# Aazmp/vp8oclenc

Hardware: AMD Instinct MI355X
Metric: macroblocks/sec inter-frame (ME+DCT+loopfilter), 1080p (higher is better)
Workload: dtype u8/int32

## Files before the change

vp8oclenc_amd/csrc/kernels_s2.hip:

```cpp
#include <stdlib.h>
#include <string.h>

#include "vp8hip_dev.h"
#include "kernels_rc_dev.h"

namespace vp8 {

namespace {

constexpr uint32_t pk8(int a, int b, int c, int d) {
    return (uint32_t)(a & 255) | ((uint32_t)(b & 255) << 8) | ((uint32_t)(c & 255) << 16) | ((uint32_t)(d & 255) << 24);
}
constexpr int TAPS[5][6] = {{3, -16, 77, 77, -16, 3}, {1, -8, 36, 108, -11, 2}, {0, 0, 128, 0, 0, 0}, {2, -11, 108, 36, -8, 1}, {3, -16, 77, 77, -16, 3}};
struct OperandTable { uint32_t w[64][4]; };
constexpr OperandTable make_bh() {
    OperandTable t{};
    for (int l = 0; l < 64; ++l) {
        const int n = l & 31, xi = n >> 3, c = n & 7, xc = xi + (xi >> 1), s = xc >= 2 ? 1 : 0;
        for (int j = 0; j < 16; ++j) {
            const int k = 16 * (l >> 5) + j, tap = k - c - s;
            const int v = k == 31 ? 64 : (tap >= 0 && tap < 6) ? TAPS[xc][tap] : 0;
            t.w[l][j >> 2] |= (uint32_t)(v & 255) << (8 * (j & 3));
        }
    }
    return t;
}
constexpr OperandTable make_av() {
    OperandTable t{};
    for (int l = 0; l < 64; ++l) {
        const int m = l & 31, f = m >> 3, i = m & 7, yc = f + (f >> 1), s = yc >= 2 ? 1 : 0;
        for (int j = 0; j < 16; ++j) {
            const int k = 16 * (l >> 5) + j, tap = k - i - s;
            const int v = k == 31 ? 64 : (tap >= 0 && tap < 6) ? TAPS[yc][tap] : 0;
            t.w[l][j >> 2] |= (uint32_t)(v & 255) << (8 * (j & 3));
        }
    }
    return t;
}
static __device__ __constant__ const OperandTable K_BH = make_bh();
static __device__ __constant__ const OperandTable K_AV = make_av();

constexpr int HT_XC = 36;
constexpr int V_CAND = 4;
constexpr int V_ROW = 26 * V_CAND;
constexpr int V_SLOT = 4 * V_ROW;
constexpr int V_ZERO = 25;
constexpr int PRE_SLOT = 96;
constexpr int WIN_ROW = 8;
__device__ __forceinline__ void lds_fence() { asm volatile("s_waitcnt lgkmcnt(0)" ::: "memory"); }

struct S2Args {
    Plane cur;
    Plane ref[3];
    const int16_t *net_in[3];
    int16_t *net_out[3];
    int32_t *bdiff[3];
    int refmap[3];
    int nrefs;
    int w, h, nblk, bw;
    uint32_t bw_inv;
    unsigned long long *clk;
};

__device__ __forceinline__ uint32_t umin(uint32_t a, uint32_t b) { return a < b ? a : b; }
template <int CTRL, int ROW_MASK = 0xf>
__device__ __forceinline__ uint32_t dpp(uint32_t v) {
    return (uint32_t)__builtin_amdgcn_update_dpp((int)v, (int)v, CTRL, ROW_MASK, 0xf, false);
}
template <int CTRL, int ROW_MASK = 0xf>
__device__ __forceinline__ uint32_t dpp_or_max(uint32_t v) {
    return (uint32_t)__builtin_amdgcn_update_dpp(-1, (int)v, CTRL, ROW_MASK, 0xf, false);
}
__device__ __forceinline__ uint32_t halfwave_min_upper(uint32_t key) {
    key = umin(key, dpp_or_max<0xb1>(key));
    key = umin(key, dpp_or_max<0x4e>(key));
    key = umin(key, dpp_or_max<0x141>(key));
    key = umin(key, dpp_or_max<0x140>(key));
    return umin(key, dpp_or_max<0x142, 0xa>(key));
}

typedef unsigned short us2 __attribute__((ext_vector_type(2)));
__device__ __forceinline__ unsigned short ashr7_pk_i8(int a, int b) { return __builtin_amdgcn_ashr_pk_i8_i32(a, b, 7); }
__device__ __forceinline__ uint32_t pack4(unsigned short lo, unsigned short hi) {
    const us2 v = {lo, hi};
    return __builtin_bit_cast(uint32_t, v);
}
__device__ __forceinline__ uint32_t round_pack4(const v16i &acc, int q) {
    return pack4(ashr7_pk_i8(acc[4 * q], acc[4 * q + 1]), ashr7_pk_i8(acc[4 * q + 2], acc[4 * q + 3]));
}
__device__ __forceinline__ v4i one_at_k31(v4i d, int upper) {
    d.w = (int)(((uint32_t)d.w & (0xffffffffu >> (8 & upper))) | (0x01000000u & (uint32_t)upper));
    return d;
}
__device__ __forceinline__ v16i mfma_round(v4i a, v4i b) {
    const v16i c = {0, 0, 0, 0, 0, 0, 0, 0, 0, 0, 0, 0, 0, 0, 0, 0};
    return __builtin_amdgcn_mfma_i32_32x32x32_i8(a, b, c, 0, 0, 0);
}

template <bool SPREAD, bool ALLREFS>
__device__ __forceinline__ void search2_body(const S2Args &a, int wg_x, int ref_idx, int tn) {
    if (ALLREFS ? a.nrefs == 0 : ref_idx >= a.nrefs) return;
    __shared__ __attribute__((aligned(16))) uint32_t s_HT[8][5 * HT_XC];
    __shared__ __attribute__((aligned(16))) uint32_t s_V[8][V_SLOT];
    uint32_t(*s_win)[V_SLOT] = s_V;
    __shared__ __attribute__((aligned(16))) int s_pre[8][PRE_SLOT];
    int(*s_q3)[5 * HT_XC] = reinterpret_cast<int(*)[5 * HT_XC]>(s_HT);
    const int g = threadIdx.x >> 5, lane = threadIdx.x & 31;
    const int wl = threadIdx.x & 63, kh = wl >> 5, gp = g & ~1;
    const int b = imin(wg_x * 8 + g, a.nblk - 1);
    const bool live = wg_x * 8 + g < a.nblk;
    const int by = a.bw == 1 ? b : (int)__umulhi((uint32_t)b, a.bw_inv), bx = b - by * a.bw;
    const int cx = bx * 8, cy = by * 8;
    {
        const int g_n = tn >> 5, lane_n = tn & 31;
        uint32_t *tmp = reinterpret_cast<uint32_t *>(&s_pre[g_n][80]);
        if (lane_n < 16) {
            const int row = lane_n >> 1, half = lane_n & 1;
            const uint32_t v = *reinterpret_cast<const uint32_t *>(a.cur.p + (ptrdiff_t)(cy + row) * a.cur.stride + cx + 4 * half) ^ 0x80808080u;
            uint8_t *cz = reinterpret_cast<uint8_t *>(tmp) + (row >> 2) * 32 + half * 16 + (row & 3);
#pragma unroll
            for (int j = 0; j < 4; ++j) cz[j * 4] = (uint8_t)(v >> (8 * j));
        }
        lds_fence();
        const int hf = lane_n & 1, t = imin(lane_n >> 1, 5), qb = imin(t, 3);
        const v4i cv = *reinterpret_cast<const v4i *>(tmp + 4 * qb);
        const uint32_t cc[4] = {(uint32_t)cv.x, (uint32_t)cv.y, (uint32_t)cv.z, (uint32_t)cv.w};
        int smcd[4], xy[4];
        weight_pre_half(cc, hf ? K_W_R2 : K_W_R0, hf ? K_W_Y : K_W_X, smcd, xy);
        int *dst = &s_pre[g_n][16 * t + 4 * hf];
        *reinterpret_cast<v4i *>(dst) = v4i{smcd[0], smcd[1], smcd[2], smcd[3]};
        *reinterpret_cast<v4i *>(dst + METRIC_X) = v4i{xy[0], xy[1], xy[2], xy[3]};
    }
    const int k = lane;
    const int dx = k % 5 - 2, dy = k / 5 - 2;
    const uint32_t kcode = k < 25 ? (uint32_t)((iabs(dx) + iabs(dy)) * 32 * 256 + (dy + 2) * 8 + dx + 2) : 40u;
    const v4i wa = metric_a(wl);

    auto one_reference = [&](int ri) {
        int tr = tn;
        if (ALLREFS) asm volatile("" : "+v"(tr));
        const int g_n = tr >> 5, lane_n = tr & 31, wl_n = tr & 63, kh_n = wl_n >> 5, gp_n = g_n & ~1;
        const int r = a.refmap[ri];
        const uint32_t nv = reinterpret_cast<const uint32_t *>(a.net_in[r])[b];
        const int nx = (int16_t)(nv & 0xffffu), ny = (int16_t)(nv >> 16);
        const int v0x = (int16_t)(nx * 4), v0y = (int16_t)(ny * 4);
        const int Lx = iclamp(cx + nx, 3 - EXT, a.w + EXT - 11), Ly = iclamp(cy + ny, 3 - EXT, a.h + EXT - 11);
        const Plane rf = a.ref[r];
        {
            const int row = lane_n >> 1, half = lane_n & 1;
            v4i v;
            __builtin_memcpy(&v, rf.p + (ptrdiff_t)(Ly - 3 + row) * rf.stride + (Lx - 3) + 16 * half, 16);
            *reinterpret_cast<v4i *>(&s_win[g_n][row * WIN_ROW + 4 * half]) = v ^ (int)0x80808080u;
        }
        const uint32_t zv = *reinterpret_cast<const uint32_t *>(rf.p + (ptrdiff_t)(cy + ((lane_n >> 1) & 7)) * rf.stride + cx + 4 * (lane_n & 1)) ^ 0x80808080u;
        lds_fence();

        {
            const int m = wl & 31, m_n = wl_n & 31;
            const v4i aw = *reinterpret_cast<const v4i *>(&s_win[gp_n + (m_n >> 4)][(m_n & 15) * WIN_ROW + 4 * kh_n]);
            const v4i bh = *reinterpret_cast<const v4i *>(K_BH.w[wl_n]);
            const v16i acc = mfma_round(one_at_k31(aw, -kh_n), bh);
            const int xi = m >> 3, c = m & 7, xc = xi + (xi >> 1);
            uint32_t *ht = &s_HT[gp][xc * HT_XC + c * 4 + kh];
#pragma unroll
            for (int q = 0; q < 4; ++q) ht[(q >> 1) * (5 * HT_XC) + 2 * (q & 1)] = round_pack4(acc, q);
        }
        {
            const int c = lane_n & 7, rg = lane_n >> 3;
            const uint8_t *wb = reinterpret_cast<const uint8_t *>(s_win[g_n]) + 3 + c + rg * (16 * WIN_ROW);
            uint32_t v = 0;
#pragma unroll
            for (int rr = 0; rr < 4; ++rr) v |= (uint32_t)wb[rr * (4 * WIN_ROW)] << (8 * rr);
            s_HT[g_n][2 * HT_XC + c * 4 + rg] = v;
        }
        {
            const int row = (lane_n >> 1) & 7, half = lane_n & 1;
            uint8_t *z = reinterpret_cast<uint8_t *>(&s_V[g_n][((row >> 2) * 2 + half) * V_ROW + V_ZERO * V_CAND]) + (row & 3);
#pragma unroll
            for (int j = 0; j < 4; ++j) z[j * 4] = (uint8_t)(zv >> (8 * j));
        }
        lds_fence();

        {
            const v4i av = *reinterpret_cast<const v4i *>(K_AV.w[wl_n]);
#pragma unroll
            for (int t = 0; t < 3; ++t) {
                const int ng = 32 * t + (wl & 31);
                const bool on = t < 2 || (wl & 31) < 16;
                const int blk = ng >= 40 ? 1 : 0, rem = on ? ng - 40 * blk : 0, xc = rem >> 3, c = rem & 7;
                const v4i hv = *reinterpret_cast<const v4i *>(&s_HT[gp + blk][xc * HT_XC + c * 4]);
                const v16i acc = mfma_round(av, one_at_k31(hv, -kh_n));
                if (on) {
                    uint32_t *sv = &s_V[gp + blk][(kh * 2 + (c >> 2)) * V_ROW + xc * V_CAND + (c & 3)];
#pragma unroll
                    for (int f = 0; f < 4; ++f) sv[(f + (f >> 1)) * 5 * V_CAND] = round_pack4(acc, f);
                    sv[2 * 5 * V_CAND] = kh ? __builtin_amdgcn_alignbyte((uint32_t)hv[2], (uint32_t)hv[1], 3)
                                            : __builtin_amdgcn_alignbyte((uint32_t)hv[1], (uint32_t)hv[0], 3);
                }
            }
        }
        lds_fence();

        int qx = (int16_t)(cx * 4 + v0x + dx), qy = (int16_t)(cy * 4 + v0y + dy);
        if (k == 25) { qx = cx * 4; qy = cy * 4; }
        const bool valid = live && k < 26 && qx >= 0 && qx <= a.w * 4 - 32 && qy >= 0 && qy <= a.h * 4 - 32;
        int diff = 0;
        auto metric = [&](const uint32_t *src, const int *pre16) { return weight_mfma(wa, load_pre16(pre16), *reinterpret_cast<const v4i *>(src)); };
        if (SPREAD) {
            int *q3 = &s_q3[g][64];
            const bool helper = lane >= 26;
            const uint32_t *src = helper ? &s_V[g][3 * V_ROW + (lane - 26) * 3 * V_CAND] : &s_V[g][k * V_CAND];
            const int step = helper ? V_CAND : V_ROW;
            const int *pre = &s_pre[g][helper ? 48 : 0];
            int *dst = &q3[helper ? (lane - 26) * 3 : 29];
#pragma unroll
            for (int j = 0; j < 3; ++j) {
                const int c = metric(src + j * step, pre + 16 * j);
                dst[j] = c;
                diff += c;
            }
            __syncthreads();
            if ((int)(threadIdx.x >> 6) == (wg_x & 3)) {
                const int slot = wl >> 3, cand = 18 + (wl & 7);
                s_q3[slot][64 + cand] = metric(&s_V[slot][3 * V_ROW + cand * V_CAND], &s_pre[slot][48]);
            }
            __syncthreads();
            diff += q3[k < 26 ? k : 31];
        } else {
            const uint32_t *src = &s_V[g][imin(k, V_ZERO) * V_CAND];
#pragma unroll
            for (int bb = 0; bb < 4; ++bb) diff += metric(src + bb * V_ROW, &s_pre[g][bb * 16]);
        }
        uint32_t key = ((uint32_t)diff << 8) + kcode;
        key = (valid && key < (0x7fffu << 8)) ? key : 0xffffffffu;
        key = halfwave_min_upper(key);
        if (lane == 16 && live) {
            int vx = (int16_t)((int16_t)(a.w * 4 - 32) - cx * 4), vy = (int16_t)((int16_t)(a.h * 4 - 32) - cy * 4), md = 0x7fff;
            if (key != 0xffffffffu) {
                const int kk = key & 0xff;
                md = (int)(key >> 8);
                vx = kk == 40 ? 0 : (int16_t)(v0x + (kk & 7) - 2);
                vy = kk == 40 ? 0 : (int16_t)(v0y + (kk >> 3) - 2);
            }
            if ((vx != 0) | (vy != 0)) md -= (iabs(vx - v0x) + iabs(vy - v0y)) * 32;
            reinterpret_cast<uint32_t *>(a.net_out[r])[b] = (uint32_t)(uint16_t)vx | ((uint32_t)(uint16_t)vy << 16);
            a.bdiff[r][b] = md;
        }
    };
    if (ALLREFS) {
#pragma unroll 1
        for (int ri = 0; ri < a.nrefs; ++ri) one_reference(ri);
    } else {
        one_reference(ref_idx);
    }
}

template <bool SPREAD, int ITER, bool ALLREFS>
__device__ __forceinline__ void search2_groups(const S2Args &a, int grp, int ref_idx) {
    if (ITER == 1 && !ALLREFS) { search2_body<SPREAD, ALLREFS>(a, grp, ref_idx, (int)threadIdx.x); return; }
#pragma unroll 1
    for (int it = 0; it < ITER; ++it) {
        int tn = (int)threadIdx.x;
        asm volatile("" : "+v"(tn));
        search2_body<SPREAD, ALLREFS>(a, grp * ITER + it, ref_idx, tn);
    }
}
template <bool SPREAD, int ITER>
__global__ __attribute__((amdgpu_waves_per_eu(7, 8))) __launch_bounds__(256) void k_search2(S2Args a) {
    launch_clock_begin(a.clk);
    search2_groups<SPREAD, ITER, false>(a, xcd_band(blockIdx.x, gridDim.x), blockIdx.y);
    launch_clock_end(a.clk);
}
static_assert(sizeof(BatchOf<S2Args>) <= 4096, "a batch's argument blocks travel in the 4 KiB kernel-argument segment");
template <bool SPREAD, int ITER>
__global__ __attribute__((amdgpu_waves_per_eu(7, 8))) __launch_bounds__(256) void k_search2_b(BatchOf<S2Args> b) {
    launch_clock_begin(b.item[0].clk);
    search2_groups<SPREAD, ITER, true>(b.item[blockIdx.z], xcd_band(blockIdx.x, gridDim.x), 0);
    launch_clock_end(b.item[0].clk);
}
struct S2Scans { rc::ScanCore item[MAX_BATCH]; uint32_t mask; int nbx, wgs; };
static_assert(sizeof(BatchOf<S2Args>) + sizeof(S2Scans) <= 4096, "the kernel-argument segment");
template <bool SPREAD, int ITER>
__global__ __attribute__((amdgpu_waves_per_eu(7, 8))) __launch_bounds__(256) void k_search2_bs(BatchOf<S2Args> b, S2Scans sc) {
    if ((int)blockIdx.x >= sc.nbx) {
        const int wg = (int)blockIdx.x - sc.nbx;
        if (((sc.mask >> blockIdx.z) & 1) && wg < sc.wgs) rc::strength_segments_body(b.item[blockIdx.z].cur, sc.item[blockIdx.z], wg, sc.wgs);
        return;
    }
    launch_clock_begin(b.item[0].clk);
    search2_groups<SPREAD, ITER, true>(b.item[blockIdx.z], xcd_band(blockIdx.x, sc.nbx), 0);
    launch_clock_end(b.item[0].clk);
}
__global__ __launch_bounds__(256, 4) void k_search2_p(BatchOf<S2Args> b, int nbx, int maxrefs, int total) {
    for (int w = blockIdx.x; w < total; w += gridDim.x) {
        const int item = w / (nbx * maxrefs), rem = w - item * (nbx * maxrefs);
        const int ref_idx = rem / nbx, wg_x = rem - ref_idx * nbx;
        search2_body<false, false>(b.item[item], wg_x, ref_idx, (int)threadIdx.x);
        lds_fence();
    }
}

}

static S2Args search2_args(const Frame &cur, const RefSet &refs, const NetSet &nets, unsigned long long *clk) {
    S2Args a;
    a.clk = clk;
    a.cur = cur.Y[0];
    int n = 0;
    for (int r = 0; r < 3; ++r) {
        a.ref[r] = refs.ref[r].Y[0];
        a.net_in[r] = nets.net[r][1];
        a.net_out[r] = nets.net[r][0];
        a.bdiff[r] = nets.bdiff[r];
        if (refs.use[r]) a.refmap[n++] = r;
    }
    a.nrefs = n;
    for (int i = n; i < 3; ++i) a.refmap[i] = 0;
    a.w = a.cur.w;
    a.h = a.cur.h;
    a.bw = a.w / 8;
    a.bw_inv = (uint32_t)(((1ull << 32) + a.bw - 1) / a.bw);
    a.nblk = a.w * a.h / 64;
    return a;
}
static bool search2_spread() {
    static const bool on = [] { const char *v = getenv("VP8HIP_S2_SPREAD"); return !(v && v[0] == '0'); }();
    return on;
}
static int search2_iter(bool batch) {
    static const int forced = [] { const char *v = getenv("VP8HIP_S2_ITER"); const int k = v && v[0] ? atoi(v) : 0; return k == 1 || k == 2 ? k : 0; }();
    return forced ? forced : (batch ? 2 : 1);
}
static bool search2_skip() {
    static const bool skip = experiment_skip("s2");
    return skip;
}

void launch_search2(hipStream_t s, const Frame &cur, const RefSet &refs, const NetSet &nets, unsigned long long *clk) {
    const S2Args a = search2_args(cur, refs, nets, clk);
    if (a.nrefs == 0 || search2_skip()) return;
    const int nbx = (a.nblk + 7) / 8;
    if (!search2_spread()) VP8_LAUNCH((k_search2<false, 1>), dim3(nbx, a.nrefs), dim3(256), 0, s, a);
    else if (search2_iter(false) == 2) VP8_LAUNCH((k_search2<true, 2>), dim3((nbx + 1) / 2, a.nrefs), dim3(256), 0, s, a);
    else VP8_LAUNCH((k_search2<true, 1>), dim3(nbx, a.nrefs), dim3(256), 0, s, a);
}

bool launch_search2_batch(hipStream_t s, const Frame *const *cur, const RefSet *refs, const NetSet *const *nets, int n, unsigned long long *clk,
                          const ScanRequest *const *scan) {
    BatchOf<S2Args> b;
    b.n = n;
    int maxrefs = 0;
    for (int i = 0; i < n; ++i) {
        b.item[i] = search2_args(*cur[i], refs[i], *nets[i], clk);
        maxrefs = b.item[i].nrefs > maxrefs ? b.item[i].nrefs : maxrefs;
    }
    if (maxrefs == 0 || search2_skip()) return false;
    const int nbx = (b.item[0].nblk + 7) / 8;
    const int persist = persistent_workgroups();
    if (persist > 0 && nbx * maxrefs * n > persist) {
        VP8_LAUNCH(k_search2_p, dim3(persist), dim3(256), 0, s, b, nbx, maxrefs, nbx * maxrefs * n);
        return false;
    }
    S2Scans sc;
    sc.mask = 0;
    for (int i = 0; scan && i < n; ++i) {
        if (!scan[i]) continue;
        const ScanRequest &q = *scan[i];
        const Plane &y = b.item[i].cur;
        sc.mask |= 1u << i;
        sc.item[i] = rc::ScanCore{q.partial, q.partial + 2 * rc::MAX_PARTIALS, q.stats, q.sd, q.strength_out,
                                  rc::SegArgs{y.w * y.h, (y.h - 1) * (y.w - 1), q.is_key, q.refqi[0], q.refqi[1], q.refqi[2], q.refqi[3], q.qi_min}};
    }
    const int iter = search2_spread() ? search2_iter(true) : 1, ngrp = (nbx + iter - 1) / iter;
    if (!sc.mask) {
        if (!search2_spread()) VP8_LAUNCH((k_search2_b<false, 1>), dim3(nbx, 1, n), dim3(256), 0, s, b);
        else if (iter == 2) VP8_LAUNCH((k_search2_b<true, 2>), dim3(ngrp, 1, n), dim3(256), 0, s, b);
        else VP8_LAUNCH((k_search2_b<true, 1>), dim3(nbx, 1, n), dim3(256), 0, s, b);
        return false;
    }
    sc.nbx = ngrp;
    sc.wgs = (b.item[0].h + rc::ROWS_PER_BLOCK - 1) / rc::ROWS_PER_BLOCK;
    if (!search2_spread()) VP8_LAUNCH((k_search2_bs<false, 1>), dim3(nbx + sc.wgs, 1, n), dim3(256), 0, s, b, sc);
    else if (iter == 2) VP8_LAUNCH((k_search2_bs<true, 2>), dim3(ngrp + sc.wgs, 1, n), dim3(256), 0, s, b, sc);
    else VP8_LAUNCH((k_search2_bs<true, 1>), dim3(nbx + sc.wgs, 1, n), dim3(256), 0, s, b, sc);
    return true;
}

}
```

Baseline: 71.90 million.

## Defer batched search2 result writes to a spread epilogue and pack validity checks

In the all-references batched path, each reference's winning key is stashed in spare LDS words of the H slot rather than written out by one lane per half-wave. After all iterations, a single epilogue spreads result decoding and global stores across many threads, one per (block, iteration, reference). The change also packs the candidate-position bounds check into 16x2 vector arithmetic, uses v_med3 for clamping, and simplifies some window-address math. It adds an extra LDS pass and recomputes block coordinates in the epilogue, and relies on the ITER<=3 assumption about spare LDS space.

```diff
diff --git a/vp8oclenc_amd/csrc/kernels_s2.hip b/vp8oclenc_amd/csrc/kernels_s2.hip
--- a/vp8oclenc_amd/csrc/kernels_s2.hip
+++ b/vp8oclenc_amd/csrc/kernels_s2.hip
@@ -46,6 +46,7 @@
 constexpr int V_SLOT = 4 * V_ROW;
 constexpr int V_ZERO = 25;
 constexpr int PRE_SLOT = 96;
+constexpr int KEY_WORD = 2 * HT_XC + 32;
 constexpr int WIN_ROW = 8;
 __device__ __forceinline__ void lds_fence() { asm volatile("s_waitcnt lgkmcnt(0)" ::: "memory"); }
 
@@ -97,10 +98,41 @@
     return __builtin_amdgcn_mfma_i32_32x32x32_i8(a, b, c, 0, 0, 0);
 }
 
+template <int LO>
+__device__ __forceinline__ int clamp_from(int v, int hi) {
+    int r;
+    asm("v_med3_i32 %0, %1, %2, %3" : "=v"(r) : "v"(v), "n"(LO), "s"(hi));
+    return r;
+}
+__device__ __forceinline__ uint32_t pk16(int lo, int hi) { return (uint32_t)(lo & 0xffff) | ((uint32_t)hi << 16); }
+__device__ __forceinline__ uint32_t pk_add(uint32_t a, uint32_t b) { return __builtin_bit_cast(uint32_t, __builtin_bit_cast(u16x2, a) + __builtin_bit_cast(u16x2, b)); }
+__device__ __forceinline__ bool qpos_valid(uint32_t nv, uint32_t pre, uint32_t last) {
+    const uint32_t q = pk_add((nv << 2) & 0xfffcfffcu, pre);
+    return __builtin_bit_cast(uint32_t, __builtin_elementwise_min(__builtin_bit_cast(u16x2, q), __builtin_bit_cast(u16x2, last))) == q;
+}
+
+__device__ __forceinline__ uint32_t s2_result(const S2Args &a, uint32_t key, uint32_t nv, int cx, int cy, int &md) {
+    const int v0x = (int16_t)((int16_t)(nv & 0xffffu) * 4), v0y = (int16_t)((int16_t)(nv >> 16) * 4);
+    int vx = (int16_t)((int16_t)(a.w * 4 - 32) - cx * 4), vy = (int16_t)((int16_t)(a.h * 4 - 32) - cy * 4);
+    md = 0x7fff;
+    if (key != 0xffffffffu) {
+        const int kk = key & 0xff;
+        md = (int)(key >> 8);
+        vx = kk == 40 ? 0 : (int16_t)(v0x + (kk & 7) - 2);
+        vy = kk == 40 ? 0 : (int16_t)(v0y + (kk >> 3) - 2);
+    }
+    if ((vx != 0) | (vy != 0)) md -= (iabs(vx - v0x) + iabs(vy - v0y)) * 32;
+    return (uint32_t)(uint16_t)vx | ((uint32_t)(uint16_t)vy << 16);
+}
+__device__ __forceinline__ uint32_t (*s2_ht())[5 * HT_XC] {
+    __shared__ __attribute__((aligned(16))) uint32_t s_HT[8][5 * HT_XC];
+    return s_HT;
+}
+
 template <bool SPREAD, bool ALLREFS>
-__device__ __forceinline__ void search2_body(const S2Args &a, int wg_x, int ref_idx, int tn) {
+__device__ __forceinline__ void search2_body(const S2Args &a, int wg_x, int ref_idx, int tn, int it = 0) {
     if (ALLREFS ? a.nrefs == 0 : ref_idx >= a.nrefs) return;
-    __shared__ __attribute__((aligned(16))) uint32_t s_HT[8][5 * HT_XC];
+    uint32_t(*s_HT)[5 * HT_XC] = s2_ht();
     __shared__ __attribute__((aligned(16))) uint32_t s_V[8][V_SLOT];
     uint32_t(*s_win)[V_SLOT] = s_V;
     __shared__ __attribute__((aligned(16))) int s_pre[8][PRE_SLOT];
@@ -134,17 +166,18 @@
     const int k = lane;
     const int dx = k % 5 - 2, dy = k / 5 - 2;
     const uint32_t kcode = k < 25 ? (uint32_t)((iabs(dx) + iabs(dy)) * 32 * 256 + (dy + 2) * 8 + dx + 2) : 40u;
-    const v4i wa = metric_a(wl);
+    const v4i wa = metric_a(tn & 63);
+    const uint32_t qpre = pk_add(pk16(cx * 4, cy * 4), k < 25 ? pk16(dx, dy) : 0u), qmax = pk16(a.w * 4 - 32, a.h * 4 - 32);
+    const bool cand = live && k < 26;
 
     auto one_reference = [&](int ri) {
         int tr = tn;
         if (ALLREFS) asm volatile("" : "+v"(tr));
-        const int g_n = tr >> 5, lane_n = tr & 31, wl_n = tr & 63, kh_n = wl_n >> 5, gp_n = g_n & ~1;
+        const int g_n = tr >> 5, lane_n = tr & 31, wl_n = tr & 63, kh_n = wl_n >> 5;
         const int r = a.refmap[ri];
         const uint32_t nv = reinterpret_cast<const uint32_t *>(a.net_in[r])[b];
         const int nx = (int16_t)(nv & 0xffffu), ny = (int16_t)(nv >> 16);
-        const int v0x = (int16_t)(nx * 4), v0y = (int16_t)(ny * 4);
-        const int Lx = iclamp(cx + nx, 3 - EXT, a.w + EXT - 11), Ly = iclamp(cy + ny, 3 - EXT, a.h + EXT - 11);
+        const int Lx = clamp_from<3 - EXT>(cx + nx, a.w + EXT - 11), Ly = clamp_from<3 - EXT>(cy + ny, a.h + EXT - 11);
         const Plane rf = a.ref[r];
         {
             const int row = lane_n >> 1, half = lane_n & 1;
@@ -156,8 +189,8 @@
         lds_fence();
 
         {
-            const int m = wl & 31, m_n = wl_n & 31;
-            const v4i aw = *reinterpret_cast<const v4i *>(&s_win[gp_n + (m_n >> 4)][(m_n & 15) * WIN_ROW + 4 * kh_n]);
+            const int m = wl & 31;
+            const v4i aw = *reinterpret_cast<const v4i *>(&s_win[gp + (m >> 4)][(m & 15) * WIN_ROW + 4 * kh]);
             const v4i bh = *reinterpret_cast<const v4i *>(K_BH.w[wl_n]);
             const v16i acc = mfma_round(one_at_k31(aw, -kh_n), bh);
             const int xi = m >> 3, c = m & 7, xc = xi + (xi >> 1);
@@ -201,10 +234,8 @@
         }
         lds_fence();
 
-        int qx = (int16_t)(cx * 4 + v0x + dx), qy = (int16_t)(cy * 4 + v0y + dy);
-        if (k == 25) { qx = cx * 4; qy = cy * 4; }
-        const bool valid = live && k < 26 && qx >= 0 && qx <= a.w * 4 - 32 && qy >= 0 && qy <= a.h * 4 - 32;
-        int diff = 0;
+        const bool valid = cand && qpos_valid(k == 25 ? 0u : nv, qpre, qmax);
+        int diff = 0, *q3k = &s_q3[g][64 + 16];
         auto metric = [&](const uint32_t *src, const int *pre16) { return weight_mfma(wa, load_pre16(pre16), *reinterpret_cast<const v4i *>(src)); };
         if (SPREAD) {
             int *q3 = &s_q3[g][64];
@@ -225,7 +256,8 @@
                 s_q3[slot][64 + cand] = metric(&s_V[slot][3 * V_ROW + cand * V_CAND], &s_pre[slot][48]);
             }
             __syncthreads();
-            diff += q3[k < 26 ? k : 31];
+            q3k = &q3[k < 26 ? k : 31];
+            diff += *q3k;
         } else {
             const uint32_t *src = &s_V[g][imin(k, V_ZERO) * V_CAND];
 #pragma unroll
@@ -234,16 +266,12 @@
         uint32_t key = ((uint32_t)diff << 8) + kcode;
         key = (valid && key < (0x7fffu << 8)) ? key : 0xffffffffu;
         key = halfwave_min_upper(key);
-        if (lane == 16 && live) {
-            int vx = (int16_t)((int16_t)(a.w * 4 - 32) - cx * 4), vy = (int16_t)((int16_t)(a.h * 4 - 32) - cy * 4), md = 0x7fff;
-            if (key != 0xffffffffu) {
-                const int kk = key & 0xff;
-                md = (int)(key >> 8);
-                vx = kk == 40 ? 0 : (int16_t)(v0x + (kk & 7) - 2);
-                vy = kk == 40 ? 0 : (int16_t)(v0y + (kk >> 3) - 2);
-            }
-            if ((vx != 0) | (vy != 0)) md -= (iabs(vx - v0x) + iabs(vy - v0y)) * 32;
-            reinterpret_cast<uint32_t *>(a.net_out[r])[b] = (uint32_t)(uint16_t)vx | ((uint32_t)(uint16_t)vy << 16);
+        if (ALLREFS) {
+            if (lane == 16) q3k[KEY_WORD - (64 + 16) + it * HT_XC + ri] = (int)key;
+        } else if (lane == 16 && live) {
+            int md;
+            const uint32_t vec = s2_result(a, key, nv, cx, cy, md);
+            reinterpret_cast<uint32_t *>(a.net_out[r])[b] = vec;
             a.bdiff[r][b] = md;
         }
     };
@@ -257,12 +285,27 @@
 
 template <bool SPREAD, int ITER, bool ALLREFS>
 __device__ __forceinline__ void search2_groups(const S2Args &a, int grp, int ref_idx) {
+    static_assert(!ALLREFS || ITER <= 3, "a group's key words are the bank skew behind x case 2 + it of the H slot (KEY_WORD): there are x cases 2, 3 and 4");
     if (ITER == 1 && !ALLREFS) { search2_body<SPREAD, ALLREFS>(a, grp, ref_idx, (int)threadIdx.x); return; }
 #pragma unroll 1
     for (int it = 0; it < ITER; ++it) {
         int tn = (int)threadIdx.x;
         asm volatile("" : "+v"(tn));
-        search2_body<SPREAD, ALLREFS>(a, grp * ITER + it, ref_idx, tn);
+        search2_body<SPREAD, ALLREFS>(a, grp * ITER + it, ref_idx, tn, it);
+    }
+    if (ALLREFS) {
+        lds_fence();
+        int tn = (int)threadIdx.x;
+        asm volatile("" : "+v"(tn));
+        const int g = tn >> 5, it = (tn >> 2) & 7, ri = tn & 3, b = (grp * ITER + it) * 8 + g;
+        if (it < ITER && ri < a.nrefs && b < a.nblk) {
+            const int r = a.refmap[ri];
+            const int by = a.bw == 1 ? b : (int)__umulhi((uint32_t)b, a.bw_inv), bx = b - by * a.bw;
+            int md;
+            const uint32_t vec = s2_result(a, s2_ht()[g][KEY_WORD + it * HT_XC + ri], reinterpret_cast<const uint32_t *>(a.net_in[r])[b], bx * 8, by * 8, md);
+            reinterpret_cast<uint32_t *>(a.net_out[r])[b] = vec;
+            a.bdiff[r][b] = md;
+        }
     }
 }
 template <bool SPREAD, int ITER>
```

Measured after the change: 73.36 million, median of 6. 2.0% higher.
